# ESMS-Group-Public/FoKL-GPy

Measured on AMD Instinct MI355X. Metric: candidate-terms/sec (basis build + Gibbs + BIC), higher is better.
Workload: dtype f64

## Files before the change

fokl_gpy_amd/_capi.py:

```python
import ctypes
import os

import numpy as np

_HERE = os.path.dirname(os.path.abspath(__file__))
LIB_PATH = os.environ.get('FOKL_HIP_LIBRARY', os.path.join(_HERE, 'libfokl_hip.so'))

UNIQUE_ID_BYTES = 128
K_BASIS, K_GRAM, K_RESID, K_PREDICT, K_RESID_MF, K_GRAM_MFMA, K_GRAM_REDUCE = 0, 1, 2, 3, 4, 5, 6
K_INTEGRATE, K_BAND = 7, 8
K_OPTIMIZE = 9
K_OPTIMIZE_SYSTEM = 10
K_POPULATION = 11
K_RESAMPLE = 12
K_SCORE = 13
K_INFER = 14
K_DESIGN = 15
INTEGRATE_MAX_STATES = 4
RESID_TERMS_MAX_FACTORS = 32
RESID_TERMS_MAX_ORDER = 8
RESID_TERMS_LAYOUTS = ((8, 1), (16, 1), (8, 2), (4, 4), (2, 8), (8, 4), (16, 2), (4, 8))
SLOT_ONES, SLOT_Y, SLOT_FIRST_FREE = 0, 1, 2
PREDICT_NONE, PREDICT_VALU_LDS, PREDICT_VALU_GLOBAL, PREDICT_MFMA = 0, 1, 2, 3
POPULATION_COEFFICIENTS = ('none', 'registers', 'table')
# ... 104 lines not shown
    'fokl_stream_given_gauss': (c_dbl, [c_vp]),
    'fokl_stream_destroy': (None, [c_vp]),
    'fokl_stream_walk': (c_int, [c_vp, c_int, c_int, c_dbl, c_dbl, c_vp, c_vp, c_vp, c_vp]),
    'fokl_stream_tell': (c_int, [c_vp, c_vp]),
    'fokl_stream_seek': (c_int, [c_vp, c_vp]),
    'fokl_stream_hold': (c_int, [c_vp, c_vp]),
    'fokl_stream_release': (c_int, [c_vp, ctypes.c_uint64]),
    'fokl_stream_advance_floor': (c_int, [c_vp]),
    'fokl_stream_state': (c_int, [c_vp, c_vp, c_vp, c_vp, c_vp]),
    'fokl_stream_expand': (c_int, [c_vp, c_int, c_dbl, c_dbl, c_vp, c_int, c_int, c_vp, c_vp, c_vp, c_vp, c_vp]),
    'fokl_stream_stats': (c_int, [c_vp, c_vp, c_vp, c_vp, c_vp, c_vp]),
    'fokl_stream_set_helpers': (c_int, [c_vp, c_int, c_vp]),
    'fokl_stream_place_bulk': (c_int, [c_vp, c_vp, c_int]),
    'fokl_stream_fast_ln_error': (c_dbl, [c_i64]),
    'fokl_search_create': (c_int, [c_vp, c_vp, c_vp, c_vp]),
    'fokl_search_bind_spectral': (c_int, [c_vp, c_vp, c_int, c_dbl, c_int]),
    'fokl_search_hold_spectral': (c_int, [c_vp, c_int]),
    'fokl_search_set_update': (c_int, [c_vp, c_int, c_int, c_int]),
    'fokl_search_set_decide': (c_int, [c_vp, c_int, c_dbl]),
    'fokl_search_set_deterministic': (c_int, [c_vp, c_int]),
    'fokl_search_destroy': (None, [c_vp]),
    'fokl_search_error': (ctypes.c_char_p, [c_vp]),
    'fokl_search_mispredicted': (c_int, [c_vp]),
    'fokl_search_set_substage': (c_int, [c_vp, c_vp, c_int]),
    'fokl_search_speculate': (c_int, [c_vp, c_vp, c_vp, c_int]),
    'fokl_search_drop_speculation': (c_int, [c_vp]),
    'fokl_search_spectral': (c_int, [c_vp, c_vp, c_int, c_vp, c_int, c_vp]),
    'fokl_search_spectral_from': (c_int, [c_vp, c_vp, c_int, c_vp, c_int, c_vp, c_int, c_vp]),
    'fokl_spectrum_done': (c_int, [c_vp]),
    'fokl_spectrum_wait': (c_int, [c_vp, c_vp, c_vp, c_vp]),
    'fokl_spectrum_release': (None, [c_vp, c_vp]),
    'fokl_spectrum_retain': (c_int, [c_vp, c_vp]),
    'fokl_search_model_begin': (c_int, [c_vp, c_vp, c_int, c_vp, c_int, c_vp, c_vp, c_vp, c_int, c_vp, c_vp]),
    'fokl_search_model_commit': (c_int, [c_vp, c_vp, c_vp, c_dbl, c_int, c_vp]),
    'fokl_run_create': (c_int, [c_vp, c_vp, c_vp]),
    'fokl_run_set_update': (c_int, [c_vp, c_int, c_int, c_int]),
    'fokl_run_search': (c_int, [c_vp, c_vp]),
    'fokl_run_result': (c_int, [c_vp, c_vp, c_vp, c_vp, c_vp, c_vp]),
    'fokl_run_arrays': (c_int, [c_vp, c_vp, c_vp, c_vp, c_vp, c_vp, c_vp]),
    'fokl_run_error': (ctypes.c_char_p, [c_vp]),
    'fokl_run_destroy': (None, [c_vp]),
    'fokl_search_score': (c_int, [c_vp, c_vp, c_dbl, c_dbl, c_int, c_int, c_vp]),
    'fokl_outcome_info': (c_int, [c_vp, c_vp, c_vp]),
    'fokl_outcome_spectrum': (c_int, [c_vp, c_vp, c_vp]),
    'fokl_outcome_chain_ready': (c_int, [c_vp]),
    'fokl_outcome_draws': (c_int, [c_vp, c_vp, c_vp]),
    'fokl_outcome_intercept_scale': (c_int, [c_vp, c_vp, c_vp]),
    'fokl_outcome_new_term_stats': (c_int, [c_vp, c_vp, c_vp, c_int, c_int, c_int, c_vp, c_vp]),
    'fokl_outcome_release': (None, [c_vp, c_vp]),
    'fokl_outcome_drop': (None, [c_vp, c_vp]),
    'fokl_search_verify': (c_int, [c_vp, c_int]),
    'fokl_search_register_forecast': (c_int, [c_vp, c_vp, c_int, c_vp, c_dbl]),
    'fokl_search_clear_forecasts': (None, [c_vp]),
    'fokl_search_likely_first_tests': (c_int, [c_vp, c_vp, c_int, c_dbl, c_vp, c_vp, c_vp]),
    'fokl_search_stats': (c_int, [c_vp, c_vp, c_int]),
    'fokl_search_trace': (c_i64, [c_vp, c_vp, c_i64]),
    'fokl_search_kill_tests': (c_int, [c_vp, c_vp, c_vp]),
    'fokl_finish_tape_blocks': (c_int, [c_int, c_int, c_vp, c_vp, c_vp, c_vp, c_int, c_int, c_int, c_vp]),
    'fokl_gibbs_chain_from_finished_tape': (c_int, [c_vp, c_vp, c_int, c_dbl, c_dbl, c_dbl, c_dbl, c_dbl, c_int, c_vp,
                                                    c_vp, c_vp, c_vp, c_int, c_vp, c_vp, c_vp, c_vp]),
    'fokl_gibbs_chain_segments_host': (c_int, [c_vp, c_vp, c_int, c_dbl, c_dbl, c_dbl, c_dbl, c_dbl, c_int, c_vp, c_vp,
                                               c_vp, c_vp, c_int, c_vp, c_vp, c_vp, c_vp, c_int, c_int, c_vp]),
    'fokl_rng_normals': (c_int, [c_vp, c_vp, c_vp, c_vp, c_i64, c_vp]),
    'fokl_rng_gammas': (c_int, [c_vp, c_vp, c_vp, c_vp, c_dbl, c_dbl, c_i64, c_vp]),
    'fokl_gp_integrate': (c_int, [c_int, c_int, c_i64, c_vp, c_vp, c_vp, c_vp, c_vp, c_vp, c_vp, c_vp, c_vp, c_int, c_int,
                                  c_dbl, c_vp, c_vp]),
    'fokl_gp_integrate_ensemble': (c_int, [c_vp, c_int, c_int, c_int, c_i64, c_vp, c_vp, c_vp, c_vp, c_vp, c_vp, c_vp, c_vp,
# ... 1284 lines not shown
    job = engine.submit(lamb, qty, b, btau, dtd, sigsqd0, tausqd0, tape, stat_first, follow=False)
    try:
        mean_w, flag = job.wait()
        return job.fetch_w(), np.array(mean_w), bool(flag[0])
    finally:
        job.release()



_OPS_SIGS = (('reserve_slots', [c_vp, c_int]),
             ('build_terms', [c_vp, c_vp, c_int, c_vp]),
             ('gram', [c_vp, c_vp, c_int, c_vp, c_int, c_vp, c_int, c_int]),
             ('gram_launch', [c_vp, c_vp, c_int, c_vp, c_int, c_int]),
             ('gram_fetch', [c_vp, c_vp, c_i64]),
             ('gram_ready', [c_vp]),
             ('bic_resid', [c_vp, c_vp, c_int, c_vp, c_vp, c_int]),
             ('bic_resid_launch', [c_vp, c_vp, c_int, c_vp]),
             ('bic_resid_fetch', [c_vp, c_vp, c_int]),
             ('bic_resid_terms_launch', [c_vp, c_vp, c_int, c_vp]))
_OPS_TYPES = {name: ctypes.CFUNCTYPE(c_int, *args) for name, args in _OPS_SIGS}


class _BackendOps(ctypes.Structure):
    _fields_ = [('ctx', c_vp)] + [(name, c_vp) for name, _ in _OPS_SIGS] + [('kernel_id', c_i32)]


class _RunParams(ctypes.Structure):
    _fields_ = [(name, c_i32) for name in (
        'm', 'n_phis', 'way3', 'tolerance', 'gimmie', 'draws', 'half0', 'lookahead', 'lookahead_native', 'foresight',
        'speculate_across', 'forecast_early', 'forecast_polls', 'matrix_free', 'update_from', 'update_depth',
        'update_lookahead', 'head_start', 'slot_capacity')]


RUN_STATS = ('terms_physical', 'substages', 'forecasts_used', 'forecasts_early', 'resid_matrix_free', 't_resid',
             'phase_prepare', 'phase_model', 'phase_statistics', 'phase_tests', 'phase_wrap_up')


def backend_ops(backend, kernel_id):
    lib = load()
    ops = _BackendOps()
    ops.kernel_id = int(kernel_id)
    ctx = getattr(backend, 'ctx', None)
    if isinstance(ctx, DeviceContext):
        ops.ctx = ctx._h
        for name, _ in _OPS_SIGS:
            setattr(ops, name, ctypes.cast(getattr(lib, 'fokl_' + name), c_vp).value)
        return ops, (ctx,)
    pending, raised = {}, []

    def arr(ptr, count, ctype, dtype):
        return np.array(np.ctypeslib.as_array(ctypes.cast(ptr, ctypes.POINTER(ctype * count)).contents), dtype=dtype)

    def guard(fn):
        def call(*args):
            try:
                fn(*args)
                return 0
            except BaseException as exc:
                raised.append(exc)
                return -3
        return call

    def out(ptr, values):
        values = np.ascontiguousarray(values, dtype=np.float64).reshape(-1)
        ctypes.memmove(ptr, values.ctypes.data, values.nbytes)

# ... 1040 lines not shown
```

fokl_gpy_amd/csrc/fokl_run.cpp:

```cpp
#include <algorithm>
#include <chrono>
#include <cmath>
#include <cstdint>
#include <cstring>
#include <map>
#include <memory>
#include <string>
#include <vector>

#include "../../include/fokl_hip_internal.h"

extern void fokl_set_global_error(const std::string &msg);

namespace {

inline double now_s()
{
    return 1e-9 * (double)std::chrono::duration_cast<std::chrono::nanoseconds>(
                      std::chrono::steady_clock::now().time_since_epoch())
                      .count();
}

using Gram = std::shared_ptr<std::vector<double>>;

// ... 219 lines not shown

struct Loop {
    fokl_run *r;
    fokl_search *s;
    const fokl_backend_ops &ops;
    const fokl_run_params &prm;
    int m;
    std::vector<int32_t> damtx;
    std::vector<int32_t> model_slots;
    std::vector<int> keep;
    Gram gram;
    int gram_A = 0;
    std::vector<int32_t> active_slots;
    int A = 0, vm = 0, n_prev = 0, vm_next = -1;
    Gram cur;
    std::vector<int32_t> terms_arr;
    int terms_pay_from = 0;
    std::map<std::vector<int64_t>, int64_t> term_ids;
    std::vector<SpectrumRef> early;
    std::vector<std::vector<int32_t>> early_keys;
    std::vector<int32_t> predicted_kills;
    bool have_predicted = false;
    Ahead ahead;
    bool have_coming = false;
    int coming_stage = 0;
    std::vector<int32_t> coming_indvec;
    struct Forecast {
        std::vector<int32_t> key;
        SpectrumRef sp;
    };
    std::vector<Forecast> forecasts;
    std::vector<fokl_outcome *> outcomes, retiring;
    int rc_cb = FOKL_OK;

    Loop(fokl_run *run, fokl_search *search) : r(run), s(search), ops(run->ops), prm(run->prm), m(run->prm.m) {}

    void release(SpectrumRef &sp)
    {
        if (sp.h) fokl_spectrum_release(s, sp.h);
        sp.h = nullptr;
        sp.gram.reset();
    }

    std::vector<int32_t> columns_without(int count, const std::vector<int32_t> &removed) const
    {
        std::vector<int32_t> out;
        for (int c = 0; c < count; ++c)
            if (std::find(removed.begin(), removed.end(), c) == removed.end()) out.push_back(c);
        return out;
    }

    int fetch_block(Ahead &a)
    {
        if (a.pending) {
            const int nc = a.over + a.T + 1;
            a.block.resize((size_t)a.T * nc);
            const int rc = ops.gram_fetch(ops.ctx, a.block.data(), (int64_t)a.T * nc);
            if (rc != FOKL_OK) return rc;
            a.pending = false;
        }
        return FOKL_OK;
    }

    int build_ahead(const std::vector<int32_t> &indvec, const std::vector<int32_t> &active, Ahead *out)
    {
        Ahead a;
        int rc = build_ahead_columns(indvec, &a);
        if (rc == FOKL_OK) rc = launch_ahead_gram(active, &a);
        if (rc != FOKL_OK) return rc;
        *out = std::move(a);
        return FOKL_OK;
    }

    int build_ahead_columns(const std::vector<int32_t> &indvec, Ahead *a)
    {
        a->vecs = arrangements(indvec);
        a->T = (int)(a->vecs.size() / (size_t)m);
        int rc = r->pool.take(a->T, &a->slots);
        if (rc != FOKL_OK) return rc;
        if ((rc = ops.build_terms(ops.ctx, a->vecs.data(), a->T, a->slots.data())) != FOKL_OK) return rc;
        r->stats[R_TERMS_PHYSICAL] += a->T;
        a->built = true;
        return FOKL_OK;
    }

    int launch_ahead_gram(const std::vector<int32_t> &active, Ahead *a)
    {
        a->over = (int)active.size();
        std::vector<int32_t> cols(active);
        cols.insert(cols.end(), a->slots.begin(), a->slots.end());
        cols.push_back(FOKL_SLOT_Y);
        const int rc = ops.gram_launch(ops.ctx, a->slots.data(), a->T, cols.data(), (int)cols.size(), 0);
        if (rc != FOKL_OK) return rc;
        a->pending = true;
        a->valid = true;
        return FOKL_OK;
    }

    void release_retired()
    {
        for (fokl_outcome *o : retiring) {
            fokl_outcome_release(s, o);
// ... 209 lines not shown
            for (int i = 0; i < n_prev; ++i) kept[(size_t)i] = i;
            cur = extend_gram(*gram, gram_A, keep, block, T, (int)cols.size(), kept, n_prev);
        }
        vm = (int)(vecs.size() / (size_t)m);
        damtx.insert(damtx.end(), vecs.begin(), vecs.end());
        const int dam = (int)(damtx.size() / (size_t)m);
        if ((rc = set_active_terms()) != FOKL_OK) return rc;
        active_slots.assign(1, FOKL_SLOT_ONES);
        active_slots.insert(active_slots.end(), model_slots.begin(), model_slots.end());
        active_slots.insert(active_slots.end(), new_slots.begin(), new_slots.end());
        A = (int)active_slots.size();
        vm_next = have_coming ? (int)(arrangements(coming_indvec).size() / (size_t)m) : -1;
        early.clear();
        early_keys.clear();
        have_predicted = false;
        bool guessed = false;
        std::vector<std::pair<int, bool>> then;
        if (vm > 0 && A > 1) then.push_back({A - 1, false});
        if (prm.lookahead > 0 && spectral_job.h && fokl_spectrum_done(spectral_job.h)) {
            if ((rc = guess_first_tests(spectral_job.h, vm, NAN, true, &then)) != FOKL_OK) return rc;
            guessed = true;
        }
        lap(R_PHASE_PREPARE);

        std::vector<int32_t> idx((size_t)A);
        for (int i = 0; i < A; ++i) idx[(size_t)i] = i;
        std::vector<int32_t> then_sizes, then_model;
        for (auto &p : then) {
            then_sizes.push_back(p.first);
            then_model.push_back(p.second ? 1 : 0);
        }
        fokl_spectrum *spectrum = nullptr;
        fokl_tape *tape = nullptr;
        if ((rc = fokl_search_model_begin(s, cur->data(), A + 1, idx.data(), A, spectral_job.h, then_sizes.data(),
                                          then_model.data(), (int)then_sizes.size(), &spectrum, &tape)) != FOKL_OK)
            return rc;
        if (g_build_at_start && have_coming && prm.foresight > 0) {
            if ((rc = build_ahead_columns(coming_indvec, &ahead)) != FOKL_OK) {
                fokl_spectrum_release(s, spectrum);
                return rc;
            }
        }
        const double *buffer = nullptr;
        int p1_check = 0;
        if ((rc = fokl_spectrum_wait(s, spectrum, &buffer, &p1_check)) != FOKL_OK) {
            fokl_spectrum_release(s, spectrum);
            return rc;
        }
        const double *betahat = buffer + 2 * (size_t)A;
        if (!terms_arr.empty() && A >= terms_pay_from) {
            rc = ops.bic_resid_terms_launch(ops.ctx, terms_arr.data() + m, A - 1, betahat);
            R->stats[R_RESID_MATRIX_FREE] += 1;
        } else {
            rc = ops.bic_resid_launch(ops.ctx, active_slots.data(), A, betahat);
        }
        if (rc == FOKL_OK && ahead.built && !ahead.valid) rc = launch_ahead_gram(active_slots, &ahead);
        if (rc == FOKL_OK && !guessed && prm.lookahead > 0 && vm > 0) {
            rc = guess_first_tests(spectrum, vm, NAN, false);
            guessed = rc == FOKL_OK;
        }
        fokl_outcome *full = nullptr;
        if (rc == FOKL_OK) rc = fokl_search_model_commit(s, spectrum, tape, (*cur)[(size_t)A * (A + 1) + A], vm, &full);
        if (rc != FOKL_OK) {
            fokl_spectrum_release(s, spectrum);
            return rc;
        }
        release(spectral_job);
        outcomes.push_back(full);
        auto forecast_now = [&]() {
            if (!(g_build_at_start && prm.forecast_early && ahead.valid && ahead.pending && have_predicted && ops.gram_ready &&
                  forecasts.empty()))
                return;
            if (!ops.gram_ready(ops.ctx)) return;
            foresee(predicted_kills.data(), (int)predicted_kills.size());
            if (rc_cb == FOKL_OK) R->stats[R_FORECASTS_EARLY] += 1;
        };
        forecast_now();
        if (rc_cb != FOKL_OK) return rc_cb;
        {
            const double t0 = now_s();
            double mom[2] = {0, 0};
            if ((rc = ops.bic_resid_fetch(ops.ctx, mom, 0)) != FOKL_OK) return rc;
            R->stats[R_T_RESID] += now_s() - t0;
            forecast_now();
            if (rc_cb != FOKL_OK) return rc_cb;
            double ev_model = 0;
            if ((rc = fokl_search_score(s, full, mom[0], mom[1], n_prev, 0, &ev_model)) != FOKL_OK) return rc;
        }
        fokl_outcome *best = full;
        fokl_outcome_view view{};
        if ((rc = fokl_outcome_info(s, full, &view)) != FOKL_OK) return rc;
        double ev = view.ev;
        lap(R_PHASE_MODEL);

        if (!guessed && prm.lookahead > 0) {
            fokl_spectrum *own = nullptr;
            if ((rc = fokl_outcome_spectrum(s, full, &own)) != FOKL_OK) return rc;
            rc = guess_first_tests(own, vm, view.siglik, false);
            fokl_spectrum_release(s, own);
            if (rc != FOKL_OK) return rc;
        }
        release_retired();
        if (have_coming && prm.foresight > 0 && !ahead.valid && !ahead.built) {
            if ((rc = build_ahead(coming_indvec, active_slots, &ahead)) != FOKL_OK) return rc;
        }
        if (prm.forecast_early && ahead.valid && ahead.pending && have_predicted && ops.gram_ready && forecasts.empty()) {
            for (int polls = prm.forecast_polls; polls > 0 && !fokl_outcome_chain_ready(full); --polls)
                if (ops.gram_ready(ops.ctx)) {
                    foresee(predicted_kills.data(), (int)predicted_kills.size());
                    if (rc_cb != FOKL_OK) return rc_cb;
                    R->stats[R_FORECASTS_EARLY] += 1;
                    break;
                }
        }
// ... 174 lines not shown
        if (r->have_next) {
            Loop head(r, nullptr);
            rc = head.build_ahead(r->next_indvec, {FOKL_SLOT_ONES}, &r->ahead);
        }
    }
    if (rc != FOKL_OK) {
        delete r;
        return rc;
    }
    *out = r;
    return FOKL_OK;
}

extern "C" int fokl_run_set_update(fokl_run *r, int from_columns, int depth, int lookahead)
{
    if (!r) return run_fail(nullptr, FOKL_ERR_ARG, "fokl_run_set_update: null run");
    r->prm.update_from = from_columns;
    r->prm.update_depth = depth;
    r->prm.update_lookahead = lookahead;
    return FOKL_OK;
}

extern "C" int fokl_run_search(fokl_run *r, fokl_search *search)
{
    if (!r || !search) return run_fail(r, FOKL_ERR_ARG, "fokl_run_search: null pointer");
    Loop loop(r, search);
    const int rc = loop.run();
    if (rc != FOKL_OK) {
        for (auto &e : loop.early) loop.release(e);
        for (auto &f : loop.forecasts) loop.release(f.sp);
        for (fokl_outcome *o : loop.outcomes) fokl_outcome_drop(search, o);
        for (fokl_outcome *o : loop.retiring) fokl_outcome_drop(search, o);
        if (loop.ahead.valid && loop.ahead.pending) (void)loop.fetch_block(loop.ahead);
    }
    return rc;
}

extern "C" int fokl_run_result(const fokl_run *r, int32_t *mtx_rows, int32_t *evs_count, int32_t *substages,
                               fokl_outcome **best_model, fokl_outcome **last_model)
{
    if (!r || !mtx_rows || !evs_count || !substages || !best_model || !last_model)
        return run_fail(nullptr, FOKL_ERR_ARG, "fokl_run_result: null pointer");
    *mtx_rows = r->mtx_rows;
    *evs_count = (int32_t)r->evs.size();
    *substages = (int32_t)r->stat_sizes.size();
    *best_model = r->best_model;
    *last_model = r->last_model;
    return FOKL_OK;
}

extern "C" int fokl_run_arrays(const fokl_run *r, int32_t *mtx, double *evs, int32_t *stat_sizes, double *stat_mean_abs,
                               double *stat_rel_std, double *stats)
{
    if (!r) return run_fail(nullptr, FOKL_ERR_ARG, "fokl_run_arrays: null run");
    if (mtx) std::memcpy(mtx, r->mtx.data(), sizeof(int32_t) * r->mtx.size());
    if (evs) std::memcpy(evs, r->evs.data(), sizeof(double) * r->evs.size());
    if (stat_sizes) std::memcpy(stat_sizes, r->stat_sizes.data(), sizeof(int32_t) * r->stat_sizes.size());
    if (stat_mean_abs) std::memcpy(stat_mean_abs, r->stat_mean_abs.data(), sizeof(double) * r->stat_mean_abs.size());
    if (stat_rel_std) std::memcpy(stat_rel_std, r->stat_rel_std.data(), sizeof(double) * r->stat_rel_std.size());
    if (stats) std::memcpy(stats, r->stats, sizeof(double) * FOKL_RUN_STATS);
    return (int)r->stat_mean_abs.size();
}

extern "C" const char *fokl_run_error(const fokl_run *r) { return r ? r->error.c_str() : ""; }

extern "C" void fokl_run_destroy(fokl_run *r)
// ... 9 lines not shown
```

fokl_gpy_amd/csrc/fokl_search.cpp:

```cpp
#include <algorithm>
#include <atomic>
#include <chrono>
#include <cmath>
#include <cstdint>
#include <cstdio>
#include <cstdlib>
#include <cstring>
#include <deque>
#include <map>
#include <memory>
#include <mutex>
#include <string>
#include <thread>
#include <vector>

#include <immintrin.h>

#include "../../include/fokl_hip_internal.h"
#include "fokl_spin.h"

extern void fokl_set_global_error(const std::string &msg);

extern "C" __attribute__((visibility("hidden"))) int fokl_gibbs_chain_from_raw_blocks(
    const double *lamb, const double *qty, int p1, double b, double btau, double dtd, double sigsqd0, double tausqd0,
// ... 1310 lines not shown
        }
        {
            const double guess = std::fabs(!std::isnan(o->ls_intercept) ? o->ls_intercept : o->spec->betahat()[0]);
            if (guess > 0.0 && !o->checks.empty())
                s->stats[S_GUESS_MAX_DEV] = std::max(s->stats[S_GUESS_MAX_DEV], std::fabs(scale / guess - 1.0));
        }
        for (const Check &c : o->checks) {
            if ((c.value < s->prm.threshav * scale) != c.decision) {
                if (s->deterministic && !block) {
                    s->misprediction_noted = true;
                    continue;
                }
                s->mispredicted = true;
                unref(s, o);
                return fail(s, FOKL_ERR_STATE,
                            "kill test decided from a guessed intercept scale that its chain does not confirm");
            }
            s->stats[S_GUESSES_VERIFIED] += 1;
        }
        o->checks.clear();
        if (o->release_wanted) release_outcome(s, o);
        unref(s, o);
    }
    if (block && s->misprediction_noted) {
        s->mispredicted = true;
        return fail(s, FOKL_ERR_STATE, "kill test decided from a guessed intercept scale or a downdated least-squares fit "
                                       "that the model's chain / eigenpairs do not confirm");
    }
    return FOKL_OK;
}

#define FOKL_SEARCH_CLONES __attribute__((target_clones("avx512f", "avx2", "default")))

FOKL_SEARCH_CLONES void inverse_from_spectrum(const double *__restrict__ Qt, const double *__restrict__ lamb, int p,
                                              double *__restrict__ inv, double *__restrict__ scaled)
{
    std::memset(inv, 0, sizeof(double) * (size_t)p * p);
    for (int e = 0; e < p; ++e) {
        const double *__restrict__ q = Qt + (size_t)e * p;
        const double w = 1.0 / lamb[e];
        for (int i = 0; i < p; ++i) scaled[i] = q[i] * w;
        for (int i = 0; i < p; ++i) {
            double *__restrict__ out = inv + (size_t)i * p;
            const double qi = scaled[i];
            for (int j = 0; j < p; ++j) out[j] += qi * q[j];
        }
    }
}

FOKL_SEARCH_CLONES void downdate_row(const double *src, const double *__restrict__ column, double f, int p, int pos,
                                     double *dst)
{
    for (int j = 0; j < pos; ++j) dst[j] = src[j] - f * column[j];
    for (int j = pos + 1; j < p; ++j) dst[j - 1] = src[j] - f * column[j];
}

struct PathModel {
    int p = 0, ld = 0;
    std::vector<int32_t> cols;
    std::vector<double> inv;
    std::vector<double> beta;
    double ssr = 0, s1 = 0;

    void init(const Spectrum *sp)
    {
        p = ld = sp->p1;
        cols.assign(sp->idx.begin(), sp->idx.end());
        beta.assign(sp->betahat(), sp->betahat() + p);
        ssr = sp->moments()[1];
        s1 = sp->moments()[0];
        if (sp->inverse.empty()) {
            sp->inverse.resize((size_t)p * p);
            std::vector<double> scaled((size_t)p);
            inverse_from_spectrum(sp->Qt(), sp->lamb(), p, sp->inverse.data(), scaled.data());
        }
        inv = sp->inverse;
    }

// ... 245 lines not shown

extern "C" int fokl_search_hold_spectral(fokl_search *s, int hold)
{
    if (!s) return fail(nullptr, FOKL_ERR_ARG, "fokl_search_hold_spectral: null search");
    s->dspec_hold = hold != 0;
    if (!s->dspec_hold) flush_spectra(s);
    return FOKL_OK;
}

extern "C" int fokl_spectrum_done(fokl_spectrum *h) { return h && spectrum_done(reinterpret_cast<Spectrum *>(h)) ? 1 : 0; }

extern "C" int fokl_spectrum_wait(fokl_search *s, fokl_spectrum *h, const double **buffer, int *p1)
{
    if (!s || !h) return fail(s, FOKL_ERR_ARG, "fokl_spectrum_wait: null pointer");
    Spectrum *sp = reinterpret_cast<Spectrum *>(h);
    const int rc = wait_spectrum(s, sp);
    if (buffer) *buffer = sp->buf;
    if (p1) *p1 = sp->p1;
    return rc;
}

extern "C" int fokl_spectrum_retain(fokl_search *s, fokl_spectrum *h)
{
    if (!s || !h) return fail(s, FOKL_ERR_ARG, "fokl_spectrum_retain: null pointer");
    reinterpret_cast<Spectrum *>(h)->refs += 1;
    return FOKL_OK;
}

extern "C" void fokl_spectrum_release(fokl_search *s, fokl_spectrum *h)
{
    if (s && h) unref(s, reinterpret_cast<Spectrum *>(h));
}

extern "C" int fokl_search_model_begin(fokl_search *s, const double *gram, int ld, const int32_t *idx, int p1,
                                       fokl_spectrum *given, const int32_t *then_sizes, const int32_t *then_model,
                                       int then_count, fokl_spectrum **spectrum_out, fokl_tape **tape_out)
{
    if (!s || !gram || !idx || p1 < 1 || !spectrum_out || !tape_out)
        return fail(s, FOKL_ERR_ARG, "fokl_search_model_begin: bad arguments");
    Tape *t = tape_for(s, p1, true);
    if (!t) return FOKL_ERR_STATE;
    std::vector<std::pair<int, bool>> want;
    for (int i = 0; i < then_count; ++i) want.push_back({then_sizes[i], then_model[i] != 0});
    speculate(s, want);
    Spectrum *sp = reinterpret_cast<Spectrum *>(given);
    if (sp)
        sp->refs += 1;
    else
        sp = submit_spectrum(s, gram, ld, idx, p1);
    if (!sp) {
        unref(s, t);
        return FOKL_ERR_STATE;
    }
    flush_spectra(s);
    const int rc = wait_spectrum(s, sp);
    if (rc != FOKL_OK) {
        unref(s, sp);
        unref(s, t);
        return rc;
    }
    *spectrum_out = reinterpret_cast<fokl_spectrum *>(sp);
    *tape_out = reinterpret_cast<fokl_tape *>(t);
    return FOKL_OK;
}

extern "C" int fokl_search_model_commit(fokl_search *s, fokl_spectrum *spectrum, fokl_tape *tape, double dtd, int new_terms,
                                        fokl_outcome **out)
{
    if (!s || !spectrum || !tape || !out || new_terms < 0)
        return fail(s, FOKL_ERR_ARG, "fokl_search_model_commit: null pointer or negative count");
    Spectrum *sp = reinterpret_cast<Spectrum *>(spectrum);
    Outcome *o = commit(s, sp, reinterpret_cast<Tape *>(tape), dtd, false, new_terms);
    unref(s, sp);
    if (!o) return FOKL_ERR_STATE;
    *out = reinterpret_cast<fokl_outcome *>(o);
    return FOKL_OK;
}

extern "C" int fokl_search_score(fokl_search *s, fokl_outcome *h, double s1, double s2, int n_prev, int kill, double *ev)
{
    if (!s || !h || !ev) return fail(s, FOKL_ERR_ARG, "fokl_search_score: null pointer");
    Outcome *o = reinterpret_cast<Outcome *>(h);
    const int p1 = o->spec->p1;
    o->ev = same_model_same_ev(s, o->spec->idx.data(), p1, ev_from_moments(s, s1, s2, p1));
    o->siglik = s->last_siglik;
    o->s1 = s1;
    o->s2 = s2;
    o->trace_index = record(s, p1, n_prev, o->ev, kill != 0);
    *ev = o->ev;
    return FOKL_OK;
}

extern "C" int fokl_outcome_info(fokl_search *s, fokl_outcome *h, fokl_outcome_view *view)
{
    if (!s || !h || !view) return fail(s, FOKL_ERR_ARG, "fokl_outcome_info: null pointer");
    Outcome *o = reinterpret_cast<Outcome *>(h);
// ... 209 lines not shown
{
    if (!s) return;
    for (auto &f : s->forecasts) unref(s, f.spec);
    s->forecasts.clear();
}

extern "C" int fokl_search_likely_first_tests(fokl_search *s, fokl_spectrum *spectrum, int n_new, double siglik,
                                              int32_t *columns_out, int32_t *accepted_out, int *count)
{
    if (!s || !spectrum || !columns_out || !count) return fail(s, FOKL_ERR_ARG, "fokl_search_likely_first_tests: null pointer");
    Spectrum *sp = reinterpret_cast<Spectrum *>(spectrum);
    const int rc = wait_spectrum(s, sp);
    if (rc != FOKL_OK) return rc;
    if (std::isnan(siglik)) siglik = sp->moments()[1] / s->prm.n - (sp->moments()[0] / s->prm.n) * (sp->moments()[0] / s->prm.n);
    const auto cols = likely_first_tests(s, sp, n_new, siglik);
    for (size_t i = 0; i < cols.size(); ++i) columns_out[i] = cols[i];
    *count = (int)cols.size();
    if (accepted_out) {
        PathModel m;
        m.init(sp);
        double ev_floor = ev_from_moments(s, m.s1, m.ssr, m.p);
        for (size_t i = 0; i < cols.size(); ++i) {
            const int at = m.position(cols[i]);
            accepted_out[i] = 0;
            if (at <= 0) continue;
            const double ev = ev_from_moments(s, m.s1, m.ssr_without(at), m.p - 1);
            if (ev < ev_floor) {
                accepted_out[i] = 1;
                ev_floor = ev;
                m.remove(at);
            }
        }
    }
    return FOKL_OK;
}

extern "C" int fokl_search_stats(const fokl_search *s, double *values, int count)
{
    if (!s || !values || count < S_COUNT) return fail(nullptr, FOKL_ERR_ARG, "fokl_search_stats: bad arguments");
    std::memcpy(values, s->stats, sizeof(double) * S_COUNT);
    return S_COUNT;
}

extern "C" int64_t fokl_search_trace(const fokl_search *s, double *records, int64_t capacity)
{
    if (!s) return 0;
    const int64_t have = (int64_t)s->trace.size() / 5;
    if (records) std::memcpy(records, s->trace.data(), sizeof(double) * 5 * (size_t)std::min(have, capacity));
    return have;
}


extern "C" int fokl_search_kill_tests(fokl_search *s, const fokl_kill_tests_args *a, fokl_kill_tests_result *res)
{
    if (!s || !a || !res || !a->gram || !a->columns || !a->mean_abs || !a->rel_std || !a->slots || !a->best ||
        !res->killed)
        return fail(s, FOKL_ERR_ARG, "fokl_search_kill_tests: null pointer");
    const double t_begin = now_s();
    const int A = a->active, ld = A + 1, vm = a->proposals;
    const double *gram = a->gram;
    const double dtd = gram[(size_t)A * ld + A];
    const double threshav = s->prm.threshav;
    Outcome *best = reinterpret_cast<Outcome *>(a->best);
    best->refs += 1;
    std::vector<char> clause1((size_t)vm);
    std::vector<int> proposal;
// ... 557 lines not shown
```

include/fokl_hip_internal.h:

```cpp
#ifndef FOKL_HIP_INTERNAL_H
#define FOKL_HIP_INTERNAL_H

#include <stddef.h>

#include "fokl_hip.h"

#ifdef __cplusplus
extern "C" {
#endif


#define FOKL_SEGMENT_BLOCKS 256
#define FOKL_SEGMENT_DOUBLES 79872
#define FOKL_ROW_LEAD (1ull << 63)
#define FOKL_SOURCE_X1_HALF (1ull << 63)
#define FOKL_SOURCE_GIVEN ((1ull << 62) - 1)
#define FOKL_GAMMA_FINAL_VALUE (~0ull)
#define FOKL_PRESTATE_WORDS 640
#define FOKL_PRESTATE_BLOCKS 32
typedef struct fokl_stream fokl_stream;
typedef struct fokl_tape_row {
    uint64_t start;
    uint64_t lead_source;
    uint64_t gamma[2];
// ... 98 lines not shown
    int32_t half0;
    int32_t aic;
    int32_t lookahead, foresight;
    int32_t speculation_max;
    int32_t tentative_tapes, test_rewinds;
    int32_t device_chain_columns;
    int32_t finish_threads;
    int32_t flip_guess;
    int32_t device_rows;
} fokl_search_params;
int fokl_search_create(fokl_host_pool *pool, fokl_dchain *dchain, const fokl_search_params *params, fokl_search **out);
typedef struct fokl_dspectral fokl_dspectral;
int fokl_search_bind_spectral(fokl_search *search, fokl_dspectral *engine, int max_columns, double slack, int lookahead);
int fokl_search_hold_spectral(fokl_search *search, int hold);
int fokl_search_set_update(fokl_search *search, int from_columns, int depth, int lookahead);
int fokl_search_set_decide(fokl_search *search, int mode, double tolerance);
int fokl_search_set_deterministic(fokl_search *search, int on);
void fokl_search_destroy(fokl_search *search);
const char *fokl_search_error(const fokl_search *search);
int fokl_search_mispredicted(const fokl_search *search);
int fokl_search_set_substage(fokl_search *search, const int64_t *term_ids, int columns);
int fokl_search_speculate(fokl_search *search, const int32_t *sizes, const int32_t *is_model, int count);
int fokl_search_drop_speculation(fokl_search *search);
int fokl_search_spectral(fokl_search *search, const double *gram, int ld, const int32_t *idx, int p1, fokl_spectrum **out);
int fokl_search_spectral_from(fokl_search *search, const double *gram, int ld, const int32_t *idx, int p1,
                              fokl_spectrum *parent, int parent_pos, fokl_spectrum **out);
int fokl_spectrum_done(fokl_spectrum *spectrum);
int fokl_spectrum_wait(fokl_search *search, fokl_spectrum *spectrum, const double **buffer, int *p1);
int fokl_spectrum_retain(fokl_search *search, fokl_spectrum *spectrum);
void fokl_spectrum_release(fokl_search *search, fokl_spectrum *spectrum);
int fokl_search_model_begin(fokl_search *search, const double *gram, int ld, const int32_t *idx, int p1,
                            fokl_spectrum *given, const int32_t *then_sizes, const int32_t *then_model, int then_count,
                            fokl_spectrum **spectrum_out, fokl_tape **tape_out);
int fokl_search_model_commit(fokl_search *search, fokl_spectrum *spectrum, fokl_tape *tape, double dtd, int new_terms,
                             fokl_outcome **out);
int fokl_search_score(fokl_search *search, fokl_outcome *outcome, double sum_r, double sum_r2, int n_prev, int kill,
                      double *ev);
typedef struct fokl_outcome_view {
    const double *spectrum;
    const int32_t *idx;
    double ev, siglik, intercept_scale;
    int32_t p1, on_device;
} fokl_outcome_view;
int fokl_outcome_info(fokl_search *search, fokl_outcome *outcome, fokl_outcome_view *view);
int fokl_outcome_spectrum(fokl_search *search, fokl_outcome *outcome, fokl_spectrum **out);
int fokl_outcome_chain_ready(fokl_outcome *outcome);
int fokl_outcome_draws(fokl_search *search, fokl_outcome *outcome, const double **w);
int fokl_outcome_intercept_scale(fokl_search *search, fokl_outcome *outcome, double *scale);
int fokl_outcome_new_term_stats(fokl_search *search, fokl_outcome *outcome, const int32_t *cols, int count, int half0,
                                int half1, double *mean_abs, double *rel_std);
void fokl_outcome_release(fokl_search *search, fokl_outcome *outcome);
void fokl_outcome_drop(fokl_search *search, fokl_outcome *outcome);
int fokl_search_verify(fokl_search *search, int block);
int fokl_search_register_forecast(fokl_search *search, const int32_t *key, int key_count, fokl_spectrum *spectrum,
                                  double dtd);
void fokl_search_clear_forecasts(fokl_search *search);
int fokl_search_likely_first_tests(fokl_search *search, fokl_spectrum *spectrum, int n_new, double siglik,
                                   int32_t *columns_out, int32_t *accepted_out, int *count);
int fokl_search_stats(const fokl_search *search, double *values, int count);
int64_t fokl_search_trace(const fokl_search *search, double *records, int64_t capacity);
typedef struct fokl_kill_tests_args {
    const double *gram;
    const int32_t *columns;
    const double *mean_abs, *rel_std;
    const int32_t *slots;
    fokl_outcome *best;
    const int32_t *ahead_keys, *ahead_offsets;
    fokl_spectrum *const *ahead_spectra;
    void *user;
    void (*foresee)(void *user, const int32_t *killed, int count);
    int (*idle_work)(void *user);
    int (*residual)(void *user, const int32_t *idx, int p1, const double *betahat, double *sum_r, double *sum_r2);
    int32_t active, proposals, n_prev, vm_next, ahead_count;
} fokl_kill_tests_args;
typedef struct fokl_kill_tests_result {
    int32_t *killed;
    fokl_outcome *best;
    double evmin;
    int32_t killed_count, best_is_new;
} fokl_kill_tests_result;
int fokl_search_kill_tests(fokl_search *search, const fokl_kill_tests_args *args, fokl_kill_tests_result *result);

typedef struct fokl_backend_ops {
    void *ctx;
    int (*reserve_slots)(void *ctx, int n_slots);
    int (*build_terms)(void *ctx, const int32_t *terms, int T, const int32_t *slots);
    int (*gram)(void *ctx, const int32_t *row_slots, int nr, const int32_t *col_slots, int nc, double *out, int path,
                int allreduce);
    int (*gram_launch)(void *ctx, const int32_t *row_slots, int nr, const int32_t *col_slots, int nc, int allreduce);
    int (*gram_fetch)(void *ctx, double *out, int64_t count);
    int (*gram_ready)(void *ctx);
// ... 389 lines not shown
```

Before: 561,600.

## Defer spectrum wait in run loop and register-block the host inverse-from-spectrum

```diff
diff --git a/fokl_gpy_amd/_capi.py b/fokl_gpy_amd/_capi.py
--- a/fokl_gpy_amd/_capi.py
+++ b/fokl_gpy_amd/_capi.py
@@ -160,7 +160,9 @@
     'fokl_spectrum_release': (None, [c_vp, c_vp]),
     'fokl_spectrum_retain': (c_int, [c_vp, c_vp]),
     'fokl_search_model_begin': (c_int, [c_vp, c_vp, c_int, c_vp, c_int, c_vp, c_vp, c_vp, c_int, c_vp, c_vp]),
+    'fokl_search_model_request': (c_int, [c_vp, c_vp, c_int, c_vp, c_int, c_vp, c_vp, c_vp, c_int, c_vp, c_vp]),
     'fokl_search_model_commit': (c_int, [c_vp, c_vp, c_vp, c_dbl, c_int, c_vp]),
+    'fokl_search_inverse_from_spectrum': (c_int, [c_vp, c_vp, c_int, c_vp, c_int]),
     'fokl_run_create': (c_int, [c_vp, c_vp, c_vp]),
     'fokl_run_set_update': (c_int, [c_vp, c_int, c_int, c_int]),
     'fokl_run_search': (c_int, [c_vp, c_vp]),
@@ -1511,6 +1513,15 @@
         'update_lookahead', 'head_start', 'slot_capacity')]
 
 
+def inverse_from_spectrum(Qt, lamb, reference=False):
+    Qt = np.ascontiguousarray(Qt, dtype=np.float64)
+    lamb = np.ascontiguousarray(lamb, dtype=np.float64)
+    p = lamb.shape[0]
+    assert Qt.shape == (p, p)
+    inv = np.empty((p, p))
+    _check(load().fokl_search_inverse_from_spectrum(_ptr(Qt), _ptr(lamb), p, _ptr(inv), int(bool(reference))))
+    return inv
+
 RUN_STATS = ('terms_physical', 'substages', 'forecasts_used', 'forecasts_early', 'resid_matrix_free', 't_resid',
              'phase_prepare', 'phase_model', 'phase_statistics', 'phase_tests', 'phase_wrap_up')
 
diff --git a/fokl_gpy_amd/csrc/fokl_run.cpp b/fokl_gpy_amd/csrc/fokl_run.cpp
--- a/fokl_gpy_amd/csrc/fokl_run.cpp
+++ b/fokl_gpy_amd/csrc/fokl_run.cpp
@@ -275,6 +275,7 @@
     std::vector<Forecast> forecasts;
     std::vector<fokl_outcome *> outcomes, retiring;
     int rc_cb = FOKL_OK;
+    bool resid_in_flight = false;
 
     Loop(fokl_run *run, fokl_search *search) : r(run), s(search), ops(run->ops), prm(run->prm), m(run->prm.m) {}
 
@@ -310,7 +311,10 @@
         Ahead a;
         int rc = build_ahead_columns(indvec, &a);
         if (rc == FOKL_OK) rc = launch_ahead_gram(active, &a);
-        if (rc != FOKL_OK) return rc;
+        if (rc != FOKL_OK) {
+            if (!a.slots.empty()) r->pool.give(a.slots);
+            return rc;
+        }
         *out = std::move(a);
         return FOKL_OK;
     }
@@ -586,8 +590,8 @@
         }
         fokl_spectrum *spectrum = nullptr;
         fokl_tape *tape = nullptr;
-        if ((rc = fokl_search_model_begin(s, cur->data(), A + 1, idx.data(), A, spectral_job.h, then_sizes.data(),
-                                          then_model.data(), (int)then_sizes.size(), &spectrum, &tape)) != FOKL_OK)
+        if ((rc = fokl_search_model_request(s, cur->data(), A + 1, idx.data(), A, spectral_job.h, then_sizes.data(),
+                                            then_model.data(), (int)then_sizes.size(), &spectrum, &tape)) != FOKL_OK)
             return rc;
         if (g_build_at_start && have_coming && prm.foresight > 0) {
             if ((rc = build_ahead_columns(coming_indvec, &ahead)) != FOKL_OK) {
@@ -608,6 +612,7 @@
         } else {
             rc = ops.bic_resid_launch(ops.ctx, active_slots.data(), A, betahat);
         }
+        resid_in_flight = rc == FOKL_OK;
         if (rc == FOKL_OK && ahead.built && !ahead.valid) rc = launch_ahead_gram(active_slots, &ahead);
         if (rc == FOKL_OK && !guessed && prm.lookahead > 0 && vm > 0) {
             rc = guess_first_tests(spectrum, vm, NAN, false);
@@ -634,6 +639,7 @@
         {
             const double t0 = now_s();
             double mom[2] = {0, 0};
+            resid_in_flight = false;
             if ((rc = ops.bic_resid_fetch(ops.ctx, mom, 0)) != FOKL_OK) return rc;
             R->stats[R_T_RESID] += now_s() - t0;
             forecast_now();
@@ -874,6 +880,13 @@
         for (fokl_outcome *o : loop.outcomes) fokl_outcome_drop(search, o);
         for (fokl_outcome *o : loop.retiring) fokl_outcome_drop(search, o);
         if (loop.ahead.valid && loop.ahead.pending) (void)loop.fetch_block(loop.ahead);
+        if (loop.resid_in_flight) {
+            double mom[2] = {0, 0};
+            (void)r->ops.bic_resid_fetch(r->ops.ctx, mom, 0);
+            loop.resid_in_flight = false;
+        }
+        if (!loop.ahead.slots.empty()) r->pool.give(loop.ahead.slots);
+        loop.ahead = Ahead();
     }
     return rc;
 }
diff --git a/fokl_gpy_amd/csrc/fokl_search.cpp b/fokl_gpy_amd/csrc/fokl_search.cpp
--- a/fokl_gpy_amd/csrc/fokl_search.cpp
+++ b/fokl_gpy_amd/csrc/fokl_search.cpp
@@ -1366,8 +1366,8 @@
 
 #define FOKL_SEARCH_CLONES __attribute__((target_clones("avx512f", "avx2", "default")))
 
-FOKL_SEARCH_CLONES void inverse_from_spectrum(const double *__restrict__ Qt, const double *__restrict__ lamb, int p,
-                                              double *__restrict__ inv, double *__restrict__ scaled)
+FOKL_SEARCH_CLONES void inverse_from_spectrum_reference(const double *__restrict__ Qt, const double *__restrict__ lamb, int p,
+                                                        double *__restrict__ inv, double *__restrict__ scaled)
 {
     std::memset(inv, 0, sizeof(double) * (size_t)p * p);
     for (int e = 0; e < p; ++e) {
@@ -1378,6 +1378,45 @@
             double *__restrict__ out = inv + (size_t)i * p;
             const double qi = scaled[i];
             for (int j = 0; j < p; ++j) out[j] += qi * q[j];
+        }
+    }
+}
+
+typedef double inv_v8 __attribute__((vector_size(64), aligned(8), may_alias));
+
+FOKL_SEARCH_CLONES void inverse_from_spectrum(const double *__restrict__ Qt, const double *__restrict__ lamb, int p,
+                                              double *__restrict__ inv, double *__restrict__ scaled)
+{
+    for (int e = 0; e < p; ++e) scaled[e] = 1.0 / lamb[e];
+    if (p < 8) {
+        for (int i = 0; i < p; ++i)
+            for (int j = 0; j < p; ++j) {
+                double acc = 0.0;
+                for (int e = 0; e < p; ++e) acc += (Qt[(size_t)e * p + i] * scaled[e]) * Qt[(size_t)e * p + j];
+                inv[(size_t)i * p + j] = acc;
+            }
+        return;
+    }
+    for (int it = 0; it < p; it += 4) {
+        const int i0 = std::min(it, p - 4);
+        for (int jt = 0; jt < p; jt += 8) {
+            const int j0 = std::min(jt, p - 8);
+            inv_v8 a0 = {0, 0, 0, 0, 0, 0, 0, 0}, a1 = a0, a2 = a0, a3 = a0;
+            const double *q = Qt;
+            for (int e = 0; e < p; ++e, q += p) {
+                const double w = scaled[e];
+                const inv_v8 qj = *reinterpret_cast<const inv_v8 *>(q + j0);
+                const double s0 = q[i0] * w, s1 = q[i0 + 1] * w, s2 = q[i0 + 2] * w, s3 = q[i0 + 3] * w;
+                a0 += s0 * qj;
+                a1 += s1 * qj;
+                a2 += s2 * qj;
+                a3 += s3 * qj;
+            }
+            double *out = inv + (size_t)i0 * p + j0;
+            *reinterpret_cast<inv_v8 *>(out) = a0;
+            *reinterpret_cast<inv_v8 *>(out + p) = a1;
+            *reinterpret_cast<inv_v8 *>(out + 2 * (size_t)p) = a2;
+            *reinterpret_cast<inv_v8 *>(out + 3 * (size_t)p) = a3;
         }
     }
 }
@@ -1689,12 +1728,12 @@
     if (s && h) unref(s, reinterpret_cast<Spectrum *>(h));
 }
 
-extern "C" int fokl_search_model_begin(fokl_search *s, const double *gram, int ld, const int32_t *idx, int p1,
-                                       fokl_spectrum *given, const int32_t *then_sizes, const int32_t *then_model,
-                                       int then_count, fokl_spectrum **spectrum_out, fokl_tape **tape_out)
+extern "C" int fokl_search_model_request(fokl_search *s, const double *gram, int ld, const int32_t *idx, int p1,
+                                         fokl_spectrum *given, const int32_t *then_sizes, const int32_t *then_model,
+                                         int then_count, fokl_spectrum **spectrum_out, fokl_tape **tape_out)
 {
     if (!s || !gram || !idx || p1 < 1 || !spectrum_out || !tape_out)
-        return fail(s, FOKL_ERR_ARG, "fokl_search_model_begin: bad arguments");
+        return fail(s, FOKL_ERR_ARG, "fokl_search_model_request: bad arguments");
     Tape *t = tape_for(s, p1, true);
     if (!t) return FOKL_ERR_STATE;
     std::vector<std::pair<int, bool>> want;
@@ -1710,15 +1749,22 @@
         return FOKL_ERR_STATE;
     }
     flush_spectra(s);
-    const int rc = wait_spectrum(s, sp);
-    if (rc != FOKL_OK) {
-        unref(s, sp);
-        unref(s, t);
-        return rc;
-    }
     *spectrum_out = reinterpret_cast<fokl_spectrum *>(sp);
     *tape_out = reinterpret_cast<fokl_tape *>(t);
     return FOKL_OK;
+}
+
+extern "C" int fokl_search_model_begin(fokl_search *s, const double *gram, int ld, const int32_t *idx, int p1,
+                                       fokl_spectrum *given, const int32_t *then_sizes, const int32_t *then_model,
+                                       int then_count, fokl_spectrum **spectrum_out, fokl_tape **tape_out)
+{
+    int rc = fokl_search_model_request(s, gram, ld, idx, p1, given, then_sizes, then_model, then_count, spectrum_out, tape_out);
+    if (rc != FOKL_OK) return rc;
+    if ((rc = wait_spectrum(s, reinterpret_cast<Spectrum *>(*spectrum_out))) != FOKL_OK) {
+        unref(s, reinterpret_cast<Spectrum *>(*spectrum_out));
+        unref(s, reinterpret_cast<Tape *>(*tape_out));
+    }
+    return rc;
 }
 
 extern "C" int fokl_search_model_commit(fokl_search *s, fokl_spectrum *spectrum, fokl_tape *tape, double dtd, int new_terms,
@@ -1994,6 +2040,17 @@
             }
         }
     }
+    return FOKL_OK;
+}
+
+extern "C" int fokl_search_inverse_from_spectrum(const double *Qt, const double *lamb, int p, double *inv, int reference)
+{
+    if (!Qt || !lamb || !inv || p < 1) return fail(nullptr, FOKL_ERR_ARG, "fokl_search_inverse_from_spectrum: bad arguments");
+    std::vector<double> scaled((size_t)p);
+    if (reference)
+        inverse_from_spectrum_reference(Qt, lamb, p, inv, scaled.data());
+    else
+        inverse_from_spectrum(Qt, lamb, p, inv, scaled.data());
     return FOKL_OK;
 }
 
diff --git a/include/fokl_hip_internal.h b/include/fokl_hip_internal.h
--- a/include/fokl_hip_internal.h
+++ b/include/fokl_hip_internal.h
@@ -154,6 +154,9 @@
 int fokl_search_model_begin(fokl_search *search, const double *gram, int ld, const int32_t *idx, int p1,
                             fokl_spectrum *given, const int32_t *then_sizes, const int32_t *then_model, int then_count,
                             fokl_spectrum **spectrum_out, fokl_tape **tape_out);
+int fokl_search_model_request(fokl_search *search, const double *gram, int ld, const int32_t *idx, int p1,
+                              fokl_spectrum *given, const int32_t *then_sizes, const int32_t *then_model, int then_count,
+                              fokl_spectrum **spectrum_out, fokl_tape **tape_out);
 int fokl_search_model_commit(fokl_search *search, fokl_spectrum *spectrum, fokl_tape *tape, double dtd, int new_terms,
                              fokl_outcome **out);
 int fokl_search_score(fokl_search *search, fokl_outcome *outcome, double sum_r, double sum_r2, int n_prev, int kill,
@@ -179,6 +182,7 @@
 void fokl_search_clear_forecasts(fokl_search *search);
 int fokl_search_likely_first_tests(fokl_search *search, fokl_spectrum *spectrum, int n_new, double siglik,
                                    int32_t *columns_out, int32_t *accepted_out, int *count);
+int fokl_search_inverse_from_spectrum(const double *Qt, const double *lamb, int p, double *inv, int reference);
 int fokl_search_stats(const fokl_search *search, double *values, int count);
 int64_t fokl_search_trace(const fokl_search *search, double *records, int64_t capacity);
 typedef struct fokl_kill_tests_args {
```

New measurement: 588,500 (median of 4 runs). 1.05x the previous value.
